# 1069066484/PanoSwinTransformerObjectDetection

Measured on AMD Instinct MI355X. Metric: panoramas/sec PanoSwin-T 512x1024 fwd+bwd, higher is better.
Workload: dtype bf16; 1 GPU; PanoSwin-T backbone (embed 96, depths 2-2-6-2, heads 3-6-12-24, ape, pano mode) fwd+bwd+AdamW on 3x512x1024 panoramas, BASELINE.json configs[1]; batch_per_gpu=8, global_batch=8, parallelism=dp1, hip_graph=True, overlap_allreduce=False, fused_window_attention=True, device=AMD Radeon Graphics

## Files before the change

### include/pswin.h

```cpp
#ifndef PSWIN_H_
#define PSWIN_H_

#include <stdint.h>

#ifdef __cplusplus
extern "C" {
#endif

#define PSWIN_ABI_VERSION 10

#define PSWIN_F32 0
#define PSWIN_BF16 1

#define PSWIN_MODE_PLANAR 0
#define PSWIN_MODE_PANO 1

#define PSWIN_OK 0
#define PSWIN_ERR_ARG (-1)
#define PSWIN_ERR_UNSUPPORTED (-2)

#define PSWIN_WS 7
#define PSWIN_WTOK 49
#define PSWIN_WPAD 64
#define PSWIN_HEAD_DIM 32
// ... 64 lines not shown
                         const float* ex_scale, int B, int S, int C, void* stream);

int pswin_ln_workspace(long long rows, int C);

int pswin_ln_partial_rows(long long rows, int C);
int pswin_ln_rows_tune(int mode);

int pswin_ln_patch_merge_fwd(const void* x, int x_dtype, const float* gamma, const float* beta, float eps, void* y,
                             int y_dtype, float* mean, float* rstd, int B, int H, int W, int C, void* stream);

int pswin_ln_patch_merge_bwd(const void* dy, int dy_dtype, const void* x, int x_dtype, const float* mean,
                             const float* rstd, const float* gamma, void* dx, float* dgamma, float* dbeta,
                             float* workspace, int B, int H, int W, int C, void* stream);

int pswin_patch_merge_gather(const void* x, int x_dtype, void* out, int out_dtype, int B, int H, int W, int C,
                             void* stream);

int pswin_patch_merge_scatter(const void* dout, int out_dtype, void* dx, int x_dtype, int B, int H, int W, int C,
                              void* stream);

int pswin_bn_workspace(int C);
int pswin_bn_relu_fwd(const void* y, int dtype, const float* gamma, const float* beta, const float* mean_offset,
                      float eps, float momentum, int train, float* running_mean, float* running_var, void* z, float* save_mean, float* save_rstd,
                      float* workspace, long long M, int C, void* stream);

int pswin_bn_relu_bwd(const void* dz, const void* y, int dtype, const float* gamma, const float* beta,
                      const float* save_mean, const float* save_rstd, int train, void* dy, float* dgamma, float* dbeta,
                      float* workspace, long long M, int C, void* stream);

int pswin_stem_workspace(int B, int H, int W);
int pswin_stem_pack_input(const float* x, int B, int H, int W, void* x4, void* stream);
int pswin_stem_conv1_stats(const void* x4, const void* w1p, int B, int H, int W, int want_xx, float* sums,
                           float* workspace, void* stream);
int pswin_stem_conv2_fwd(const void* x4, const void* w1p, const float* scale1, const float* shift1, const void* w2p, int B,
                         int H, int W, void* y2, float* sums2, float* workspace, void* stream);
int pswin_stem_conv3_fwd(const void* y2, const float* scale2, const float* shift2, const void* w3p, const float* bias3,
                         int B, int H, int W, void* tokens, void* stream);

int pswin_stem_conv3_bwd_stats(const void* dtok, const void* y2, const float* prm, const void* w3t, int B, int H, int W,
                               float* sums, float* workspace, void* stream);
int pswin_stem_conv3_bwd_data(const void* dtok, const void* y2, const float* prm, const void* w3t, int B, int H, int W,
                              void* dy2, void* stream);
int pswin_stem_conv3_wgrad(const void* dtok, const void* y2, const float* scale2, const float* shift2, int B, int H, int W,
                           const int32_t* perm, float* dw3, float* workspace, void* stream);
int pswin_stem_conv2_wgrad(const void* x4, const void* w1p, const float* scale1, const float* shift1, const void* dy2, int B,
                           int H, int W, const int32_t* perm, float* dw2, float* workspace, void* stream);
int pswin_stem_conv2_bwd(const void* x4, const void* w1p, const float* prm, const void* dy2, const void* w2t, int B, int H,
                         int W, float* out, float* workspace, void* stream);

int pswin_bias_gelu_fwd(const void* y, int dtype, const float* bias, void* h, long long M, int N, void* stream);
int pswin_bias_gelu_workspace(long long M, int N);
int pswin_bias_gelu_tune(int unr_fwd, int unr_bwd);
int pswin_bias_gelu_partial_rows(long long M, int N, int dtype);
int pswin_bias_gelu_bwd(const void* dh, const void* y, int dtype, const float* bias, void* dy, float* dbias,
                        float* workspace, long long M, int N, void* stream);

int pswin_stem_pack_weights(const float* w1, const float* w2, const float* w3, void* w1p, void* w2p, void* w2t, void* w3p,
                            void* w3t, void* stream);
int pswin_stem_bn_fold(const float* sum, const float* sumsq, double count, const float* gamma, const float* beta,
                       const float* conv_bias, float eps, float momentum, int training, float* running_mean,
                       float* running_var, int C, float* prm, long long* num_batches_tracked, void* stream);
int pswin_stem_bn2_coefs(const float* sums, const float* prm, double count, int training, float* prm5, void* stream);
int pswin_stem_conv1_wgrad(const float* out5, const float* xx, const void* w1p, const float* prm1, double count, int training,
                           float* dw1, float* db1, void* stream);

int pswin_gemm_tn_ring_supported(long long M, int N, int K);
int pswin_gemm_tn_ring_splits(long long M, int N, int K, int target_wgs);
int pswin_gemm_tn_ring(const void* dy, const void* x, void* partial, int partial_dtype, long long M, int N, int K, int splits, void* stream);
int pswin_gemm_tn_ring_bias(const void* dy, const void* x, void* partial, int partial_dtype, float* dbias_partial, int zero_lo, int zero_hi,
                            long long M, int N, int K, int splits, void* stream);

typedef struct pswin_tn_job {
    const void* dy;
    const void* x;
    void* partial;
    float* dbias_partial;
    long long M;
    int N, K, splits, partial_dtype, zero_lo, zero_hi;
    const float* sample_scale;
    int rows_per_sample;
} pswin_tn_job;
int pswin_gemm_tn_ring_jobs(const pswin_tn_job* jobs, int n_jobs, void* stream);
int pswin_gemm_tn_ring_table_bytes(void);

typedef struct pswin_transpose_job {
    const void* src;
    void* dst;
    int rows;
    int cols;
} pswin_transpose_job;
int pswin_transpose_jobs(const pswin_transpose_job* jobs, int n_jobs, void* stream);

int pswin_adamw_flat(float* p, const float* g, float* m, float* v, void* p_bf16, long long n, double lr, double beta1, double beta2, double eps,
                     double weight_decay, const float* step, void* stream);
#define PSWIN_ADAMW_MAX_GROUPS 8
int pswin_adamw_flat_groups(float* p, const float* g, float* m, float* v, void* p_bf16, long long n, const unsigned char* group_of,
                            int n_groups, const float* lr_mult, const float* decay_mult, double lr, double beta1, double beta2, double eps,
                            double weight_decay, const float* step, void* stream);

#define PSWIN_LR_FIXED 0
#define PSWIN_LR_STEP 1
#define PSWIN_WARMUP_NONE 0
#define PSWIN_WARMUP_CONSTANT 1
#define PSWIN_WARMUP_LINEAR 2
#define PSWIN_WARMUP_EXP 3
#define PSWIN_LR_MAX_MILESTONES 8
#define PSWIN_GRADSQ_PARTIALS 1024
typedef struct pswin_lr_schedule {
    int policy;
    int warmup;
    int warmup_iters;
    int by_epoch;
    int iters_per_epoch;
    int n_milestones;
    int step_every;
    int has_min_lr;
    int milestones[PSWIN_LR_MAX_MILESTONES];
    double warmup_ratio;
    double gamma;
    double min_lr;
} pswin_lr_schedule;
typedef struct pswin_step_record {
    double lr[PSWIN_ADAMW_MAX_GROUPS];
    double norm;
    float lr_base;
    float norm_f;
    float coef;
    float t;
    int applied;
    int iteration;
} pswin_step_record;
int pswin_grad_sumsq(const float* g, long long n, double* partials, void* stream);
int pswin_adamw_record(const double* partials, const pswin_lr_schedule* sched, double lr, int n_groups, const float* lr_mult,
                       double max_norm, int skip_nonfinite, float* step, float* iteration, float* skipped, pswin_step_record* record,
                       void* stream);
int pswin_adamw_flat_sched(float* p, const float* g, float* m, float* v, void* p_bf16, long long n, const unsigned char* group_of,
                           int n_groups, const float* decay_mult, double beta1, double beta2, double eps, double weight_decay,
                           const pswin_step_record* record, void* stream);
#define PSWIN_ROI_MAX_LEVELS 4
typedef struct pswin_roi_levels {
    const void* feat[PSWIN_ROI_MAX_LEVELS];
    float* dfeat[PSWIN_ROI_MAX_LEVELS];
    int H[PSWIN_ROI_MAX_LEVELS];
    int W[PSWIN_ROI_MAX_LEVELS];
    float spatial_scale[PSWIN_ROI_MAX_LEVELS];
    int n_levels;
} pswin_roi_levels;
int pswin_roi_align_supported(int C, int dtype);
int pswin_roi_align_fwd(const pswin_roi_levels* levels, const float* rois, const int32_t* roi_level, int R, int C, int P, int sampling_ratio,
                        int aligned, int dtype, void* out, void* stream);
int pswin_roi_align_bwd(const pswin_roi_levels* levels, const float* rois, const int32_t* roi_level, int R, int C, int P, int sampling_ratio,
                        int aligned, int dtype, const void* dout, void* stream);

int pswin_nms_workspace(int groups, int nmax);
int pswin_nms_groups(const float* boxes, const int32_t* counts, int groups, int nmax, float iou_threshold, unsigned char* keep, void* workspace,
                     void* stream);

int pswin_max_iou_assign_rows_per_workgroup(void);
int pswin_max_iou_assign_workspace(int B, int N, int Gmax);
int pswin_max_iou_assign(const float* cand, int cand_per_image, const float* gt, const int32_t* gt_count, int B, int N, int Gmax, int lead_gt,
                         float pos_iou_thr, float neg_iou_thr, float min_pos_iou, int match_low_quality, long long* gt_inds, float* max_iou,
                         void* workspace, void* stream);

int pswin_gemm_nt_supported(long long M, int K, int N);
int pswin_gemm_nt(const void* x, const void* w, const float* bias, void* y, long long M, int K, int N, int tile_m, void* stream);
int pswin_gemm_nt_f32(const void* x, const void* w, const float* bias, float* y, long long M, int K, int N, int tile_m, void* stream);
// ... 283 lines not shown
```

### panoswintransformerobjectdetection_amd/_lib.py

```python
import ctypes
import os

import torch

_PKG = os.path.dirname(os.path.abspath(__file__))
LIB_PATH = os.environ.get("PSWIN_LIB") or os.path.join(_PKG, "libpswin_hip.so")

F32, BF16 = 0, 1
MODE_PLANAR, MODE_PANO = 0, 1
WS, WTOK, WPAD, HEAD_DIM = 7, 49, 64, 32
ABI_VERSION = 10

_vp, _i, _f = ctypes.c_void_p, ctypes.c_int, ctypes.c_float
_ip = ctypes.POINTER(ctypes.c_int)

_PROTOTYPES = {
    "pswin_version": [],
    "pswin_window_grid": [_i, _i, _i, _ip, _ip, _ip],
    "pswin_window_map": [_i, _i, _i, _i, _vp, _vp, _vp],
    "pswin_planar_mask": [_i, _i, _i, _vp, _vp],
    "pswin_uv_grid": [_i, _i, _vp, _vp],
    "pswin_abs_pos_features": [_vp, _i, _vp, _vp],
    "pswin_gather_uv": [_vp, _vp, _i, _vp, _vp],
    "pswin_haversine_windows": [_vp, _vp, _i, _vp, _vp],
    "pswin_window_gather": [_vp, _i, _vp, _vp, _vp, _i, _i, _i, _i, _i, _vp],
    "pswin_window_scatter_add": [_vp, _i, _vp, _vp, _vp, _vp, _vp, _i, _i, _i, _i, _i, _vp],
    "pswin_ln_gather_fwd": [_vp, _i, _vp, _vp, _vp, _f, _vp, _i, _vp, _vp, _i, _i, _i, _i, _vp],
    "pswin_ln_gather_fwd_add": [_vp, _i, _vp, _vp, _vp, _f, _vp, _vp, _i, _vp, _vp, _i, _i, _i, _i, _vp],
    "pswin_ln_gather_bwd": [_vp, _i, _vp, _vp, _i, _vp, _vp, _vp, _vp, _vp, _vp, _vp, _vp, _vp, _vp, _i, _i, _i, _i, _vp],
    "pswin_ln_gather_bwd_ex": [_vp, _i, _vp, _vp, _i, _vp, _vp, _vp, _vp, _vp, _vp, _vp, _vp, _vp, _vp, _i, _i, _i, _i, _vp, _vp, _i, _vp, _vp, _i,
                               _vp],
    "pswin_scatter_add_ln_fwd": [_vp, _i, _vp, _vp, _vp, _vp, _vp, _vp, _vp, _f, _vp, _i, _vp, _vp, _i, _i, _i, _i, _vp],
    "pswin_scatter_add_ln_fwd_map": [_vp, _i, _vp, _vp, _vp, _vp, _vp, _vp, _vp, _f, _vp, _i, _vp, _vp, _i, _i, _i, _i, _vp, _i, _vp, _i, _vp],
    "pswin_ln_nchw_supported": [_i, _i],
    "pswin_ln_nchw_fwd": [_vp, _vp, _vp, _f, _vp, _vp, _vp, _i, _i, _i, _vp],
    "pswin_ln_nchw_bwd": [_vp, _vp, _vp, _vp, _vp, _vp, _vp, _vp, _vp, _vp, _i, _i, _i, _vp],
    "pswin_scatter_add_ln_nchw_fwd": [_vp, _vp, _vp, _vp, _vp, _vp, _vp, _f, _vp, _vp, _vp, _i, _i, _i, _vp],
    "pswin_ln_nchw_bwd_ex": [_vp, _vp, _vp, _vp, _vp, _vp, _vp, _vp, _vp, _vp, _vp, _vp, _i, _i, _i, _vp],
    "pswin_ln_workspace": [ctypes.c_longlong, _i],
    "pswin_ln_patch_merge_fwd": [_vp, _i, _vp, _vp, _f, _vp, _i, _vp, _vp, _i, _i, _i, _i, _vp],
    "pswin_ln_patch_merge_bwd": [_vp, _i, _vp, _i, _vp, _vp, _vp, _vp, _vp, _vp, _vp, _i, _i, _i, _i, _vp],
    "pswin_patch_merge_gather": [_vp, _i, _vp, _i, _i, _i, _i, _i, _vp],
    "pswin_patch_merge_scatter": [_vp, _i, _vp, _i, _i, _i, _i, _i, _vp],
    "pswin_bn_workspace": [_i],
    "pswin_bn_relu_fwd": [_vp, _i, _vp, _vp, _vp, _f, _f, _i, _vp, _vp, _vp, _vp, _vp, _vp, ctypes.c_longlong, _i, _vp],
    "pswin_bn_relu_bwd": [_vp, _vp, _i, _vp, _vp, _vp, _vp, _i, _vp, _vp, _vp, _vp, ctypes.c_longlong, _i, _vp],
    "pswin_stem_workspace": [_i, _i, _i],
    "pswin_stem_pack_input": [_vp, _i, _i, _i, _vp, _vp],
    "pswin_stem_conv1_stats": [_vp, _vp, _i, _i, _i, _i, _vp, _vp, _vp],
    "pswin_stem_conv2_fwd": [_vp, _vp, _vp, _vp, _vp, _i, _i, _i, _vp, _vp, _vp, _vp],
    "pswin_stem_conv3_fwd": [_vp, _vp, _vp, _vp, _vp, _i, _i, _i, _vp, _vp],
    "pswin_stem_conv3_bwd_stats": [_vp, _vp, _vp, _vp, _i, _i, _i, _vp, _vp, _vp],
    "pswin_stem_conv3_bwd_data": [_vp, _vp, _vp, _vp, _i, _i, _i, _vp, _vp],
    "pswin_stem_conv3_wgrad": [_vp, _vp, _vp, _vp, _i, _i, _i, _vp, _vp, _vp, _vp],
    "pswin_stem_conv2_wgrad": [_vp, _vp, _vp, _vp, _vp, _i, _i, _i, _vp, _vp, _vp, _vp],
    "pswin_stem_conv2_bwd": [_vp, _vp, _vp, _vp, _vp, _i, _i, _i, _vp, _vp, _vp],
    "pswin_stem_pack_weights": [_vp, _vp, _vp, _vp, _vp, _vp, _vp, _vp, _vp],
    "pswin_stem_bn_fold": [_vp, _vp, ctypes.c_double, _vp, _vp, _vp, _f, _f, _i, _vp, _vp, _i, _vp, _vp, _vp],
    "pswin_stem_bn2_coefs": [_vp, _vp, ctypes.c_double, _i, _vp, _vp],
    "pswin_stem_conv1_wgrad": [_vp, _vp, _vp, _vp, ctypes.c_double, _i, _vp, _vp, _vp],
    "pswin_gemm_tn_ring_supported": [ctypes.c_longlong, _i, _i],
    "pswin_gemm_tn_ring_splits": [ctypes.c_longlong, _i, _i, _i],
    "pswin_gemm_tn_ring": [_vp, _vp, _vp, _i, ctypes.c_longlong, _i, _i, _i, _vp],
    "pswin_gemm_tn_ring_bias": [_vp, _vp, _vp, _i, _vp, _i, _i, ctypes.c_longlong, _i, _i, _i, _vp],
    "pswin_gemm_tn_ring_jobs": [_vp, _i, _vp],
    "pswin_gemm_tn_ring_table_bytes": [],
    "pswin_transpose_jobs": [_vp, _i, _vp],
    "pswin_adamw_flat": [_vp, _vp, _vp, _vp, _vp, ctypes.c_longlong, ctypes.c_double, ctypes.c_double, ctypes.c_double, ctypes.c_double, ctypes.c_double, _vp, _vp],
    "pswin_adamw_flat_groups": [_vp, _vp, _vp, _vp, _vp, ctypes.c_longlong, _vp, _i, _vp, _vp, ctypes.c_double, ctypes.c_double,
                                ctypes.c_double, ctypes.c_double, ctypes.c_double, _vp, _vp],
    "pswin_grad_sumsq": [_vp, ctypes.c_longlong, _vp, _vp],
    "pswin_adamw_record": [_vp, _vp, ctypes.c_double, _i, _vp, ctypes.c_double, _i, _vp, _vp, _vp, _vp, _vp],
    "pswin_adamw_flat_sched": [_vp, _vp, _vp, _vp, _vp, ctypes.c_longlong, _vp, _i, _vp, ctypes.c_double, ctypes.c_double, ctypes.c_double,
                               ctypes.c_double, _vp, _vp],
    "pswin_roi_align_supported": [_i, _i],
    "pswin_roi_align_fwd": [_vp, _vp, _vp, _i, _i, _i, _i, _i, _i, _vp, _vp],
    "pswin_roi_align_bwd": [_vp, _vp, _vp, _i, _i, _i, _i, _i, _i, _vp, _vp],
    "pswin_nms_workspace": [_i, _i],
    "pswin_nms_groups": [_vp, _vp, _i, _i, ctypes.c_float, _vp, _vp, _vp],
    "pswin_max_iou_assign_rows_per_workgroup": [],
    "pswin_max_iou_assign_workspace": [_i, _i, _i],
    "pswin_max_iou_assign": [_vp, _i, _vp, _vp, _i, _i, _i, _i, _f, _f, _f, _i, _vp, _vp, _vp, _vp],
    "pswin_multiclass_nms_scores": [_vp, _i, _vp, _i, _i, _i, _f, _vp, _vp],
    "pswin_multiclass_nms_workspace": [_i, _i, _i],
    "pswin_multiclass_nms": [_vp, _vp, _vp, _vp, _i, _vp, _i, _i, _vp, _i, _i, _i, _f, _vp, _vp, _vp],
    "pswin_multiclass_nms_select": [_vp, _vp, ctypes.c_longlong, _i, _vp, _vp, _i, _vp, _i, _i, _vp, _i, _i, _i, _i, _vp, _vp, _vp, _vp, _vp, _vp],
    "pswin_paste_masks": [_vp, _i, ctypes.c_longlong, ctypes.c_longlong, ctypes.c_longlong, ctypes.c_longlong, _vp, _vp, _vp, _i, _i, _i, _i, _i,
                          _f, _vp, _vp],
    "pswin_aug_merge_proposals_launches": [_i, _i, _i],
    "pswin_aug_merge_proposals_workspace": [_i, _i, _i, _i],
    "pswin_aug_merge_proposals": [_vp, _vp, _vp, _vp, _i, _i, _i, _f, _i, _vp, _vp, _vp, _vp, _vp],
    "pswin_aug_map_rois": [_vp, _vp, _i, _i, _i, _vp, _vp],
    "pswin_aug_merge_bboxes": [_vp, _vp, _vp, _i, _i, _vp, _vp, _i, _i, _i, _i, _vp, _vp, _vp],
    "pswin_multiclass_nms_scores_boxes": [_vp, _vp, _i, _i, _i, _f, _vp, _vp],
    "pswin_multiclass_nms_boxes": [_vp, _vp, _vp, _i, _i, _i, _f, _vp, _vp, _vp],
    "pswin_multiclass_nms_select_boxes": [_vp, _vp, ctypes.c_longlong, _i, _vp, _i, _i, _i, _i, _vp, _vp, _vp, _vp, _vp, _vp],
    "pswin_paste_masks_aug": [_vp, _i, _vp, _vp, _vp, _i, _i, _i, _i, _i, _f, _vp, _vp],
    "pswin_rle_workspace": [ctypes.c_longlong, _i, _i, _vp],
    "pswin_rle_encode": [_vp, _vp, ctypes.c_longlong, _i, _i, _i, _vp, _vp, ctypes.c_longlong, _vp, _vp],
    "pswin_paste_masks_rle": [_vp, _i, ctypes.c_longlong, ctypes.c_longlong, ctypes.c_longlong, ctypes.c_longlong, _vp, _vp, _vp, _i, _i, _i, _i,
                              _i, _f, _vp, _vp, ctypes.c_longlong, _vp, _vp],
    "pswin_sample_rows_per_workgroup": [],
    "pswin_sample_workspace": [_i, _i, _i],
    "pswin_sample_ranks": [_vp, _vp, _i, _i, _i, _i, _vp, _vp, _vp, _vp],
    "pswin_rpn_targets": [_vp, _vp, _vp, _vp, _vp, _i, _i, _i, _i, _i, _vp, _vp, _vp, _vp, _vp],
    "pswin_roi_targets": [_vp, _vp, _vp, _vp, _vp, _vp, _i, _i, _i, _i, _i, _i, _vp, _vp, _vp, _vp, _vp, _vp, _vp],
    "pswin_mask_targets": [_vp, _vp, _vp, _vp, _i, _i, _i, _i, _i, _i, _vp, _vp],
    "pswin_rpn_proposals_rows_per_workgroup": [],
    "pswin_rpn_proposals_launches": [_vp, _i, _i, _i],
    "pswin_rpn_proposals_workspace": [_vp, _i, _i, _i, _i],
    "pswin_rpn_proposals": [_vp, _vp, _vp, _vp, _i, _i, _i, _f, _i, _i, _i, _vp, _vp, _vp, _vp, _vp],
    "pswin_cascade_rows_per_workgroup": [],
    "pswin_cascade_refine": [_vp, _vp, _i, _vp, _i, _vp, _i, _i, _i, _vp, _i, _i, _vp, _vp, _vp],
    "pswin_giou_rows_fwd": [_vp, _vp, _i, _vp, _vp, _vp, _i, _i, _vp, ctypes.c_double, _vp, _vp],
    "pswin_giou_rows_bwd": [_vp, _vp, _i, _vp, _vp, _vp, _vp, _i, _i, _vp, ctypes.c_double, _vp, _vp],
    "pswin_losses_rows_per_workgroup": [],
    "pswin_rpn_losses_chunk": [],
    "pswin_ce_rows_fwd": [_vp, _i, _vp, _i, _i, _vp, _vp],
    "pswin_ce_rows_bwd": [_vp, _i, _vp, _vp, _i, _i, _vp, _vp],
    "pswin_l1_rows_fwd": [_vp, _i, _vp, _vp, _vp, _i, _i, _vp, _vp],
    "pswin_l1_rows_bwd": [_vp, _i, _vp, _vp, _vp, _vp, _i, _i, _vp, _vp],
    "pswin_mask_bce_rows_fwd": [_vp, _i, ctypes.c_longlong, ctypes.c_longlong, ctypes.c_longlong, ctypes.c_longlong, _vp, _vp, _vp, _i, _i, _i,
                                _vp, _vp, _vp],
    "pswin_mask_bce_rows_bwd": [_vp, _i, ctypes.c_longlong, ctypes.c_longlong, ctypes.c_longlong, ctypes.c_longlong, _vp, _vp, _vp, _vp, _i, _i,
                                _i, _vp, _vp],
    "pswin_rpn_losses_fwd": [_vp, _vp, _vp, _vp, _vp, _vp, _i, _i, _i, _i, _vp, _vp],
    "pswin_rpn_losses_bwd": [_vp, _vp, _vp, _vp, _vp, _vp, _vp, _i, _i, _i, _i, _vp, _vp, _vp],
    "pswin_ap_segments_chunk": [],
    "pswin_box_iou_pairs": [_vp, _vp, _vp, _vp, _vp, _vp, _i, _i, _i, _vp, _vp, _vp, _vp],
    "pswin_mask_iou_workspace": [_i, _i, _i],
    "pswin_mask_iou_pairs": [_vp, _vp, _vp, _vp, _vp, _vp, _i, _i, _i, _i, _i, _vp, _vp, _vp, _vp, _vp],
    "pswin_eval_match": [_vp, _vp, _vp, _vp, _vp, _vp, _vp, _vp, _vp, _vp, _i, _vp, _i, _i, _i, _i, _i, _i, _vp, _vp, _vp, _vp, _vp, _vp, _vp,
                         _vp],
    "pswin_ap_segments": [_vp, _vp, _vp, _i, _i, _i, ctypes.c_longlong, _vp, _vp],
    "pswin_recall_match": [_vp, _vp, _vp, _vp, _vp, _vp, _i, _vp, _i, _i, _i, _i, _vp, _vp, _vp, _vp],
    "pswin_mask_inter_pairs": [_vp, _vp, _vp, _vp, _vp, _vp, _i, _i, _i, _i, _i, _vp, _vp, _vp],
    "pswin_coco_supported": [_i, _i, _i, _i, _i, _i],
    "pswin_coco_accumulate_chunk": [],
    "pswin_coco_match": [_vp, _vp, _vp, _vp, _vp, _vp, _vp, _vp, _vp, _vp, _vp, _vp, _i, _vp, _i, _i, _i, _i, _i, _i, _vp, _vp, _vp, _vp, _vp,
                         _vp, _vp, _vp, _vp],
    "pswin_coco_accumulate": [_vp, _vp, _vp, _vp, _vp, _i, _vp, _i, _i, _i, _i, ctypes.c_longlong, _vp, _vp, _vp],
    "pswin_gemm_nt_supported": [ctypes.c_longlong, _i, _i],
    "pswin_gemm_nt": [_vp, _vp, _vp, _vp, ctypes.c_longlong, _i, _i, _i, _vp],
    "pswin_gemm_nt_f32": [_vp, _vp, _vp, _vp, ctypes.c_longlong, _i, _i, _i, _vp],
    "pswin_gemm_nt_gelu_fwd": [_vp, _vp, _vp, _vp, _vp, ctypes.c_longlong, _i, _i, _i, _vp],
    "pswin_gemm_nt_partial_rows": [ctypes.c_longlong, _i],
    "pswin_gemm_nt_gelu_bwd": [_vp, _vp, _vp, _vp, _vp, _vp, ctypes.c_longlong, _i, _i, _i, _vp],
    "pswin_gemm_nt_live": [_vp, _vp, _vp, _vp, ctypes.c_longlong, _i, _i, _i, _vp, _i, _vp],
    "pswin_gemm_nt_gelu_fwd_live": [_vp, _vp, _vp, _vp, _vp, ctypes.c_longlong, _i, _i, _i, _vp, _i, _vp],
# ... 208 lines not shown
```

### panoswintransformerobjectdetection_amd/csrc/pswin_gemm_tn.hip

```cpp
#include <type_traits>

#include "pswin_common.hpp"

using namespace pswin;

namespace {

constexpr int MSTEP = 64, PANEL = 64 * 64 * 2;
using rsrc_t = __amdgpu_buffer_rsrc_t;
typedef __attribute__((address_space(3))) void lds_void;

constexpr int RING_THREADS = 512;
template <int WK, int WN, int STAGES>
struct RingGeom {
    static constexpr int PX = (96 * WK + 63) / 64, PD = (48 * WN + 63) / 64, PANELS = PX + PD, STAGE_BYTES = PANELS * PANEL;
    static constexpr int LOADS = PANELS;
    static constexpr int XWAVES = PX;
    static_assert(WK * WN == 8, "eight waves");
    static_assert((size_t)STAGES * STAGE_BYTES <= 160 * 1024, "LDS");
};

template <int OFF>
__device__ inline void ds_tr(u32x2& dst, unsigned addr) {
    asm volatile("ds_read_b64_tr_b16 %0, %1 offset:%2" : "=v"(dst) : "v"(addr), "i"(OFF) : "memory");
}
struct Frag {
    u32x2 lo, hi;
};
__device__ inline bf16x8 frag_bf16(const Frag& f) { return __builtin_bit_cast(bf16x8, u32x4{f.lo[0], f.lo[1], f.hi[0], f.hi[1]}); }
__device__ inline void wait_frags(Frag (&a)[6], Frag (&b)[3]) {
    asm volatile("s_waitcnt lgkmcnt(0)"
                 : "+v"(a[0].lo), "+v"(a[0].hi), "+v"(a[1].lo), "+v"(a[1].hi), "+v"(a[2].lo), "+v"(a[2].hi), "+v"(a[3].lo), "+v"(a[3].hi),
                   "+v"(a[4].lo), "+v"(a[4].hi), "+v"(a[5].lo), "+v"(a[5].hi), "+v"(b[0].lo), "+v"(b[0].hi), "+v"(b[1].lo), "+v"(b[1].hi),
                   "+v"(b[2].lo), "+v"(b[2].hi)
                 :
                 : "memory");
}

struct TnJob {
    const unsigned short* dy;
    const unsigned short* x;
    void* part;
    float* db;
    const float* sample_scale;
    int M, N, K, rows_per_split, zero_lo, zero_hi;
    int first_wg, flags, xmap, rows_per_sample;
};
constexpr int TN_JOBS_MAX = 48;
struct TnBatch {
    TnJob job[TN_JOBS_MAX];
    int n;
};
static_assert(sizeof(TnJob) == 80 && sizeof(TnBatch) <= 4000, "the job table travels in the 4 KB kernel-argument segment");

template <int WK, int WN, int STAGES>
__global__ __launch_bounds__(RING_THREADS, 2) void gemm_tn_ring_kernel(const TnBatch batch) {
    using G = RingGeom<WK, WN, STAGES>;
    int jlo = 0, jhi = batch.n - 1;
    while (jlo < jhi) {
        const int mid = (jlo + jhi + 1) >> 1;
        if (batch.job[mid].first_wg <= (int)blockIdx.x) jlo = mid;
        else jhi = mid - 1;
    }
    const TnJob& job = batch.job[jlo];
    const int jbid = (int)blockIdx.x - job.first_wg;
    const unsigned short* __restrict__ DY = job.dy;
    const unsigned short* __restrict__ X = job.x;
    void* __restrict__ P = job.part;
    float* __restrict__ DB = job.db;
    const int M = job.M, N = job.N, K = job.K, rows_per_split = job.rows_per_split;
    const int tiles_k = (K + 96 * WK - 1) / (96 * WK), tiles_n = (N + 48 * WN - 1) / (48 * WN);
    const int zero_lo = job.zero_lo, zero_hi = job.zero_hi;
    const bool out_bf16 = (job.flags & 1) != 0;
    constexpr int IA = 6, JB = 3;
    constexpr int RING_STAGE_BYTES = G::STAGE_BYTES, LOADS = G::LOADS;
    extern __shared__ __attribute__((aligned(1024))) char smem[];
    const int tid = threadIdx.x;
    const int wave = __builtin_amdgcn_readfirstlane(tid >> 6), lane = tid & 63;
    const int c = lane & 15, g = lane >> 4;
    const int wk = wave / WN, wn = wave - wk * WN;

    int split, tk, tn;
    {
        const int xm = job.xmap, g = xm & 255, gn = (xm >> 8) & 255, bk = (xm >> 16) & 255, bn = (xm >> 24) & 255;
        const int xcd = jbid & 7, loc = jbid >> 3, lane = xcd / g, blk = xcd - lane * g, ik = blk / gn, in = blk - ik * gn;
        const int per = bk * bn, round = loc / per, within = loc - round * per, wk_ = within / bn;
        split = round * (8 / g) + lane;
        tk = ik * bk + wk_;
        tn = in * bn + (within - wk_ * bn);
        if (split >= (job.flags >> 1) || tk >= tiles_k || tn >= tiles_n) return;
    }
    const int k0 = tk * (96 * WK), n0 = tn * (48 * WN);
    const int m_begin = split * rows_per_split;
    int steps = rows_per_split / MSTEP;
    {
        const int left = (M - m_begin + MSTEP - 1) / MSTEP;
        steps = left < steps ? (left > 0 ? left : 0) : steps;
    }
    const float* __restrict__ SS = job.sample_scale;
    unsigned long long live_slabs = 0ull;
    if (SS != nullptr) {
        const int rows_per_sample = job.rows_per_sample;
        const unsigned long long live_samples = live_sample_mask(SS, M / rows_per_sample);
        bool live = false;
        if (lane < steps) {
            const int r0 = m_begin + lane * MSTEP, r1 = (r0 + MSTEP < M ? r0 + MSTEP : M) - 1;
            const int s0 = r0 / rows_per_sample, s1 = r1 / rows_per_sample;
            const unsigned long long span = s1 - s0 >= 63 ? ~0ull : (2ull << (s1 - s0)) - 1ull;
            live = ((live_samples >> s0) & span) != 0ull;
        }
        const unsigned long long b = __ballot(live);
        live_slabs = (unsigned long long)(unsigned)__builtin_amdgcn_readfirstlane((int)(unsigned)b) |
                     (unsigned long long)(unsigned)__builtin_amdgcn_readfirstlane((int)(unsigned)(b >> 32)) << 32;
        steps = __builtin_popcountll(live_slabs);
    }

    static_assert((G::PX * 8) % LOADS == 0, "a wave's blocks must not straddle the two operands");
    const bool mine_x = wave * LOADS < G::PX * 8;
    const rsrc_t src = mine_x ? __builtin_amdgcn_make_buffer_rsrc(const_cast<unsigned short*>(X), 0, (int)((size_t)M * K * 2), 0x00020000)
                              : __builtin_amdgcn_make_buffer_rsrc(const_cast<unsigned short*>(DY), 0, (int)((size_t)M * N * 2), 0x00020000);
    const unsigned ld2 = (unsigned)((mine_x ? K : N) * 2);
    const int c0 = mine_x ? k0 : n0;
    const int lr = lane >> 3, pch = lane & 7;
    unsigned goff[8];
    const int last_panel = ((mine_x ? K : N) - c0 + 63) / 64 - 1;
#pragma unroll
    for (int j = 0; j < LOADS; ++j) {
        const int blk_all = wave * LOADS + j - (mine_x ? 0 : G::PX * 8), blk = blk_all & 7;
        int panel = blk_all >> 3;
        panel = panel > last_panel ? (last_panel > 0 ? last_panel : 0) : panel;
        const int row = 8 * blk + lr;
        const int f = ((row >> 1) & 1) | (((row >> 3) & 1) << 1);
        const int col = (((pch >> 1) ^ f) << 4) + ((pch & 1) << 3);
        goff[j] = (unsigned)row * ld2 + (unsigned)((c0 + 64 * panel + col) * 2);
    }
    auto issue = [&](int step, int stage) {
        char* base = smem + stage * RING_STAGE_BYTES + wave * LOADS * 1024;
        int slab = step;
        if (SS != nullptr) {
            slab = __builtin_ctzll(live_slabs);
            live_slabs &= live_slabs - 1ull;
        }
        const unsigned m = (unsigned)(m_begin + slab * MSTEP) * ld2;
#pragma unroll
        for (int j = 0; j < LOADS; ++j) __builtin_amdgcn_raw_ptr_buffer_load_lds(src, (lds_void*)(base + j * 1024), 16, goff[j] + m, 0, 0, 0);
    };

    f32x4 acc[IA][JB];
#pragma unroll
    for (int i = 0; i < IA; ++i)
#pragma unroll
        for (int j = 0; j < JB; ++j) acc[i][j] = f32x4{0.f, 0.f, 0.f, 0.f};
    const bool sum_db = DB != nullptr && tk == 0 && wk == 0;
    f32x4 accs[JB];
#pragma unroll
    for (int j = 0; j < JB; ++j) accs[j] = f32x4{0.f, 0.f, 0.f, 0.f};
    const bf16x8 ones = __builtin_bit_cast(bf16x8, u32x4{0x3F803F80u, 0x3F803F80u, 0x3F803F80u, 0x3F803F80u});

    const int q = c >> 2, p8 = c & 3;
    const int fl = ((q >> 1) & 1) | ((g & 1) << 1);
    const unsigned lds0 = (unsigned)(size_t)(lds_void*)smem;
    const unsigned lane_row = lds0 + (unsigned)((8 * g + q) * 128 + p8 * 8);
    unsigned xoff[4];
#pragma unroll
    for (int cb = 0; cb < 4; ++cb) xoff[cb] = ((unsigned)(cb ^ fl) << 5) + lane_row;
    unsigned abase[IA], bbase[JB];
#pragma unroll
    for (int i = 0; i < IA; ++i) {
        const int col0 = wk * 96 + 16 * i;
        abase[i] = xoff[(col0 >> 4) & 3] + (unsigned)((col0 >> 6) * PANEL);
    }
#pragma unroll
    for (int j = 0; j < JB; ++j) {
        const int col0 = wn * 48 + 16 * j;
        bbase[j] = xoff[(col0 >> 4) & 3] + (unsigned)((col0 >> 6) * PANEL + G::PX * PANEL);
    }
    auto read_n = [&](auto ks_tag, auto n_tag, unsigned stage_off, Frag (&a)[6], Frag (&b)[3]) {
        constexpr int KS = decltype(ks_tag)::value, NN = decltype(n_tag)::value, F = NN >> 1, OFF = KS * 4096 + (NN & 1) * 512;
        if constexpr (F < 6) {
            if constexpr (NN & 1) ds_tr<OFF>(a[F].hi, abase[F] + stage_off);
            else ds_tr<OFF>(a[F].lo, abase[F] + stage_off);
        } else {
            if constexpr (NN & 1) ds_tr<OFF>(b[F - 6].hi, bbase[F - 6] + stage_off);
            else ds_tr<OFF>(b[F - 6].lo, bbase[F - 6] + stage_off);
        }
    };
    auto mma_n = [&](auto n_tag, const bf16x8 (&af)[6], const bf16x8 (&bfr)[3]) {
        constexpr int NN = decltype(n_tag)::value, I = NN % 6, J = NN / 6;
        acc[I][J] = mfma32(af[I], bfr[J], acc[I][J]);
    };
    auto phase = [&](auto ks_tag, auto read_tag, unsigned stage_off, Frag (&cur_a)[6], Frag (&cur_b)[3], Frag (&nxt_a)[6], Frag (&nxt_b)[3]) {
        constexpr bool READ = decltype(read_tag)::value;
        bf16x8 af[IA], bfr[JB];
#pragma unroll
        for (int i = 0; i < IA; ++i) af[i] = frag_bf16(cur_a[i]);
#pragma unroll
        for (int j = 0; j < JB; ++j) bfr[j] = frag_bf16(cur_b[j]);
        auto slot = [&](auto n_tag) {
            if constexpr (READ) read_n(ks_tag, n_tag, stage_off, nxt_a, nxt_b);
            mma_n(n_tag, af, bfr);
            __builtin_amdgcn_sched_barrier(0);
        };
        [&]<int... Ns>(std::integer_sequence<int, Ns...>) { (slot(std::integral_constant<int, Ns>{}), ...); }(std::make_integer_sequence<int, 18>{});
        if (sum_db) {
#pragma unroll
            for (int j = 0; j < JB; ++j) accs[j] = mfma32(ones, bfr[j], accs[j]);
        }
    };
    auto read_all = [&](auto ks_tag, unsigned stage_off, Frag (&a)[6], Frag (&b)[3]) {
        [&]<int... Ns>(std::integer_sequence<int, Ns...>) { (read_n(ks_tag, std::integral_constant<int, Ns>{}, stage_off, a, b), ...); }(std::make_integer_sequence<int, 18>{});
    };
    using KS0 = std::integral_constant<int, 0>;
    using KS1 = std::integral_constant<int, 1>;

    static_assert(STAGES == 2 || STAGES == 3, "");
    static_assert(STAGES == 2 || LOADS == 6, "the counted wait below is written out for 6 loads per slab");
    if (steps > 0) issue(0, 0);
    if (STAGES == 3 && steps > 1) issue(1, 1);
    Frag a0[6], b0[3], a1[6], b1[3];
    int stage = 0;
    for (int st = 0; st < steps; ++st) {
        if (STAGES == 3 && st + 1 < steps) asm volatile("s_waitcnt vmcnt(6)" ::: "memory");
        else asm volatile("s_waitcnt vmcnt(0)" ::: "memory");
        if (st > 0) wait_frags(a1, b1);
        __builtin_amdgcn_s_barrier();
        const unsigned stage_off = (unsigned)(stage * RING_STAGE_BYTES);
        if (st + STAGES - 1 < steps) issue(st + STAGES - 1, stage == 0 ? STAGES - 1 : stage - 1);
        if (st == 0) {
            read_all(KS0{}, stage_off, a0, b0);
        } else {
            phase(KS0{}, std::true_type{}, stage_off, a1, b1, a0, b0);
        }
        wait_frags(a0, b0);
        __builtin_amdgcn_sched_barrier(0);
        phase(KS1{}, std::true_type{}, stage_off, a0, b0, a1, b1);
        stage = stage == STAGES - 1 ? 0 : stage + 1;
    }
    if (steps > 0) {
        wait_frags(a1, b1);
        __builtin_amdgcn_sched_barrier(0);
        phase(KS0{}, std::false_type{}, 0u, a1, b1, a0, b0);
    }

    if (sum_db && g == 0) {
#pragma unroll
        for (int j = 0; j < JB; ++j) {
            const int n = n0 + wn * 48 + 16 * j + c;
            if (n < N) DB[(size_t)split * N + n] = (n >= zero_lo && n < zero_hi) ? 0.f : accs[j][0];
        }
    }
#pragma unroll
    for (int j = 0; j < JB; ++j) {
        const int n = n0 + wn * 48 + 16 * j + c;
        if (n >= N) continue;
#pragma unroll
        for (int i = 0; i < IA; ++i) {
            const int k = k0 + wk * 96 + 16 * i + 4 * g;
            if (k >= K) continue;
            const size_t o = (size_t)split * N * K + (size_t)n * K + k;
            if (out_bf16) {
                *reinterpret_cast<u32x2*>(reinterpret_cast<unsigned short*>(P) + o) = u32x2{pack2_bf16(acc[i][j][0], acc[i][j][1]), pack2_bf16(acc[i][j][2], acc[i][j][3])};
            } else {
                *reinterpret_cast<f32x4*>(reinterpret_cast<float*>(P) + o) = acc[i][j];
            }
        }
    }
}

inline int ring_geom(int N, int K) {
    if (N >= 192 && K >= 192 && N % 192 == 0 && K % 192 == 0) return 0;
    if (K == 96 && N >= 48 && N <= 384 && N % 16 == 0) return 1;
    if (K == 384 && N == 96) return 2;
    return -1;
}

template <int WK, int WN, int STAGES>
int launch_tn_batch(const TnBatch& b, int wgs, hipStream_t st) {
    using G = RingGeom<WK, WN, STAGES>;
    constexpr size_t lds = (size_t)STAGES * G::STAGE_BYTES;
    static std::atomic<unsigned long long> configured{0};
    if (const int rc = ensure_dynamic_lds(reinterpret_cast<const void*>(&gemm_tn_ring_kernel<WK, WN, STAGES>), lds, configured)) return rc;
    hipLaunchKernelGGL((gemm_tn_ring_kernel<WK, WN, STAGES>), dim3(wgs), dim3(RING_THREADS), lds, st, b);
    PSWIN_LAUNCH_RET();
}

inline bool tn_job_ok(const pswin_tn_job& q) {
    return q.dy && q.x && q.partial && q.M >= 64 && (q.M + 64) * (long long)(q.K > q.N ? q.K : q.N) * 2 < 0xFFFFFF00ll && ring_geom(q.N, q.K) >= 0 &&
           q.splits >= 1 && q.splits <= q.M / 64 && valid_dtype(q.partial_dtype) && aligned16(q.dy) && aligned16(q.x) && aligned16(q.partial) &&
           q.zero_lo >= 0 && q.zero_hi >= q.zero_lo && q.zero_hi <= q.N &&
           (!q.sample_scale || (q.rows_per_sample > 0 && q.M % q.rows_per_sample == 0 && q.M / q.rows_per_sample <= LIVE_SAMPLES_MAX &&
                                (q.M + q.splits - 1) / q.splits <= 64 * MSTEP));
}

int launch_tn_jobs(const pswin_tn_job* jobs, int n_jobs, int geom, hipStream_t st) {
    TnBatch b;
    b.n = 0;
    long long wgs = 0;
    auto flush = [&]() -> int {
        if (b.n == 0) return PSWIN_OK;
        int rc;
        if (geom == 0) rc = launch_tn_batch<2, 4, 3>(b, (int)wgs, st);
        else if (geom == 1) rc = launch_tn_batch<1, 8, 2>(b, (int)wgs, st);
        else rc = launch_tn_batch<4, 2, 2>(b, (int)wgs, st);
        b.n = 0;
        wgs = 0;
        return rc;
    };
    for (int i = 0; i < n_jobs; ++i) {
        const pswin_tn_job& q = jobs[i];
        if (ring_geom(q.N, q.K) != geom) continue;
        const int tk = geom == 0 ? 192 : (geom == 1 ? 96 : 384), tn = geom == 0 ? 192 : (geom == 1 ? 384 : 96);
        TnJob& j = b.job[b.n];
        j.dy = reinterpret_cast<const unsigned short*>(q.dy);
        j.x = reinterpret_cast<const unsigned short*>(q.x);
        j.part = q.partial;
        j.db = q.dbias_partial;
        j.M = (int)q.M;
        j.N = q.N;
        j.K = q.K;
        const int tiles_k = (q.K + tk - 1) / tk, tiles_n = (q.N + tn - 1) / tn;
        j.sample_scale = q.sample_scale;
        j.rows_per_sample = q.sample_scale ? q.rows_per_sample : 0;
        j.rows_per_split = (int)(((q.M + q.splits - 1) / q.splits + MSTEP - 1) / MSTEP * MSTEP);
        j.zero_lo = q.zero_lo;
        j.zero_hi = q.zero_hi;
        j.first_wg = (int)wgs;
        int n_wg;
        {
            const int S = q.splits;
            int g = 1;
            if (S < 8) {
                int p2 = 1;
                while (p2 < S) p2 *= 2;
                g = 8 / p2;
            }
            int best_gn = 1;
            long long best = -1;
            for (int gn = 1; gn <= g; gn *= 2) {
                const int gk = g / gn;
                const long long cost = (long long)((tiles_k + gk - 1) / gk) * tk + (long long)((tiles_n + gn - 1) / gn) * tn;
                if (best < 0 || cost < best) best = cost, best_gn = gn;
            }
            const int gn = best_gn, gk = g / gn, bk = (tiles_k + gk - 1) / gk, bn = (tiles_n + gn - 1) / gn;
            const int lanes = 8 / g, rounds = (S + lanes - 1) / lanes;
            j.xmap = g | gn << 8 | bk << 16 | bn << 24;
            n_wg = 8 * rounds * bk * bn;
        }
        j.flags = (q.partial_dtype == PSWIN_BF16 ? 1 : 0) | q.splits << 1;
        wgs += n_wg;
        if (++b.n == TN_JOBS_MAX || wgs > (1ll << 24)) {
            if (const int rc = flush()) return rc;
        }
    }
    return flush();
}

}

extern "C" {

int pswin_gemm_tn_ring_supported(long long M, int N, int K) {
    return M >= 64 && (M + 64) * (long long)(K > N ? K : N) * 2 < 0xFFFFFF00ll && ring_geom(N, K) >= 0;
}

int pswin_gemm_tn_ring_splits(long long M, int N, int K, int target_wgs) {
    if (!pswin_gemm_tn_ring_supported(M, N, K)) return PSWIN_ERR_ARG;
    const int geom = ring_geom(N, K);
    const int tiles = geom == 0 ? (N / 192) * (K / 192) : 1;
    if (target_wgs <= 0) target_wgs = 256;
    int s = target_wgs / tiles;
    const int smax = (int)(M / 256) > 0 ? (int)(M / 256) : 1;
    if (s > smax) s = smax;
    return s < 1 ? 1 : s;
}

int pswin_gemm_tn_ring_table_bytes(void) { return (int)sizeof(TnBatch); }

int pswin_gemm_tn_ring_jobs(const pswin_tn_job* jobs, int n_jobs, void* stream) {
    PSWIN_CHECK_ARG(jobs && n_jobs > 0);
    for (int i = 0; i < n_jobs; ++i) PSWIN_CHECK_ARG(tn_job_ok(jobs[i]));
    for (int geom = 0; geom < 3; ++geom)
        if (const int rc = launch_tn_jobs(jobs, n_jobs, geom, (hipStream_t)stream)) return rc;
    return PSWIN_OK;
}

int pswin_gemm_tn_ring_bias(const void* dy, const void* x, void* partial, int partial_dtype, float* dbias_partial, int zero_lo, int zero_hi, long long M,
                            int N, int K, int splits, void* stream) {
    pswin_tn_job q;
    q.dy = dy;
    q.x = x;
    q.partial = partial;
    q.dbias_partial = dbias_partial;
    q.M = M;
    q.N = N;
    q.K = K;
    q.splits = splits;
    q.partial_dtype = partial_dtype;
    q.zero_lo = zero_lo;
    q.zero_hi = zero_hi;
    q.sample_scale = nullptr;
    q.rows_per_sample = 0;
    return pswin_gemm_tn_ring_jobs(&q, 1, stream);
}

int pswin_gemm_tn_ring(const void* dy, const void* x, void* partial, int partial_dtype, long long M, int N, int K, int splits, void* stream) {
    return pswin_gemm_tn_ring_bias(dy, x, partial, partial_dtype, nullptr, 0, 0, M, N, K, splits, stream);
}

}
```

Measured before the change: 885.7 panoramas/s.

## Merge all wgrad ring geometries into one launch with job reordering

Replaces the per-geometry template kernels with a single kernel that dispatches on geometry packed into each job's xmap, so all TN wgrad jobs go out in one launch instead of up to three. Jobs are sorted by rows per split, longest first. An optional env-gated mode splits the work into two queues and interleaves them by proportional block share. A host-side plan API is added for inspection. In exchange, every geometry now reserves the largest LDS ring and the fused kernel may hold more registers, which can lower occupancy for the smaller geometries.

```diff
diff --git a/include/pswin.h b/include/pswin.h
--- a/include/pswin.h
+++ b/include/pswin.h
@@ -170,6 +170,7 @@
 } pswin_tn_job;
 int pswin_gemm_tn_ring_jobs(const pswin_tn_job* jobs, int n_jobs, void* stream);
 int pswin_gemm_tn_ring_table_bytes(void);
+int pswin_gemm_tn_ring_plan(const pswin_tn_job* jobs, int n_jobs, int interleave, int* plan, int cap, int* n_launches);
 
 typedef struct pswin_transpose_job {
     const void* src;
diff --git a/panoswintransformerobjectdetection_amd/_lib.py b/panoswintransformerobjectdetection_amd/_lib.py
--- a/panoswintransformerobjectdetection_amd/_lib.py
+++ b/panoswintransformerobjectdetection_amd/_lib.py
@@ -65,6 +65,7 @@
     "pswin_gemm_tn_ring_bias": [_vp, _vp, _vp, _i, _vp, _i, _i, ctypes.c_longlong, _i, _i, _i, _vp],
     "pswin_gemm_tn_ring_jobs": [_vp, _i, _vp],
     "pswin_gemm_tn_ring_table_bytes": [],
+    "pswin_gemm_tn_ring_plan": [_vp, _i, _i, _vp, _i, _vp],
     "pswin_transpose_jobs": [_vp, _i, _vp],
     "pswin_adamw_flat": [_vp, _vp, _vp, _vp, _vp, ctypes.c_longlong, ctypes.c_double, ctypes.c_double, ctypes.c_double, ctypes.c_double, ctypes.c_double, _vp, _vp],
     "pswin_adamw_flat_groups": [_vp, _vp, _vp, _vp, _vp, ctypes.c_longlong, _vp, _i, _vp, _vp, ctypes.c_double, ctypes.c_double,
diff --git a/panoswintransformerobjectdetection_amd/csrc/pswin_gemm_tn.hip b/panoswintransformerobjectdetection_amd/csrc/pswin_gemm_tn.hip
--- a/panoswintransformerobjectdetection_amd/csrc/pswin_gemm_tn.hip
+++ b/panoswintransformerobjectdetection_amd/csrc/pswin_gemm_tn.hip
@@ -1,4 +1,8 @@
+#include <algorithm>
+#include <cstdlib>
+#include <cstring>
 #include <type_traits>
+#include <vector>
 
 #include "pswin_common.hpp"
 
@@ -43,35 +47,64 @@
     void* part;
     float* db;
     const float* sample_scale;
-    int M, N, K, rows_per_split, zero_lo, zero_hi;
-    int first_wg, flags, xmap, rows_per_sample;
+    int M, N, K, splits, zero_lo, zero_hi;
+    int first_wg, xmap;
 };
-constexpr int TN_JOBS_MAX = 48;
+__host__ __device__ inline int tn_xmap(int lg, int lgn, int geom, int out_bf16, int samples, int bk, int bn) {
+    return lg | lgn << 2 | geom << 4 | out_bf16 << 6 | samples << 7 | bk << 16 | bn << 24;
+}
+__host__ __device__ inline int tn_rows_per_split(int M, int splits) { return ((M + splits - 1) / splits + MSTEP - 1) / MSTEP * MSTEP; }
+__host__ __device__ inline int tn_tile_k(int geom) { return geom == 0 ? 192 : (geom == 1 ? 96 : 384); }
+__host__ __device__ inline int tn_tile_n(int geom) { return geom == 0 ? 192 : (geom == 1 ? 384 : 96); }
+
+constexpr int TN_JOBS_MAX = 54;
 struct TnBatch {
     TnJob job[TN_JOBS_MAX];
-    int n;
+    int n, n0, blocks0, blocks1;
+    unsigned share;
 };
-static_assert(sizeof(TnJob) == 80 && sizeof(TnBatch) <= 4000, "the job table travels in the 4 KB kernel-argument segment");
-
-template <int WK, int WN, int STAGES>
-__global__ __launch_bounds__(RING_THREADS, 2) void gemm_tn_ring_kernel(const TnBatch batch) {
-    using G = RingGeom<WK, WN, STAGES>;
-    int jlo = 0, jhi = batch.n - 1;
+static_assert(sizeof(TnJob) == 72 && sizeof(TnBatch) <= 4000, "the job table travels in the 4 KB kernel-argument segment");
+
+__host__ __device__ inline int tn_queue1_before(int b, int blocks0, int blocks1, unsigned share) {
+    const long long h = (long long)(((unsigned long long)(unsigned)b * share + 32768ull) >> 16), lo = b - blocks0;
+    const long long c = h < lo ? lo : h;
+    return (int)(c > blocks1 ? blocks1 : c);
+}
+__host__ __device__ inline int tn_find_job(const TnBatch& batch, int wg, int& jbid) {
+    const int b = wg >> 3;
+    const int h0 = tn_queue1_before(b, batch.blocks0, batch.blocks1, batch.share), h1 = tn_queue1_before(b + 1, batch.blocks0, batch.blocks1, batch.share);
+    const bool q1 = h1 != h0;
+    const int qwg = (q1 ? h0 : b - h0) << 3 | (wg & 7);
+    int jlo = q1 ? batch.n0 : 0, jhi = (q1 ? batch.n : batch.n0) - 1;
     while (jlo < jhi) {
         const int mid = (jlo + jhi + 1) >> 1;
-        if (batch.job[mid].first_wg <= (int)blockIdx.x) jlo = mid;
+        if (batch.job[mid].first_wg <= qwg) jlo = mid;
         else jhi = mid - 1;
     }
-    const TnJob& job = batch.job[jlo];
-    const int jbid = (int)blockIdx.x - job.first_wg;
+    jbid = qwg - batch.job[jlo].first_wg;
+    return jlo;
+}
+__host__ __device__ inline bool tn_slot(int xm, int splits, int tiles_k, int tiles_n, int jbid, int& split, int& tk, int& tn) {
+    const int g = 1 << (xm & 3), gn = 1 << ((xm >> 2) & 3), bk = (xm >> 16) & 255, bn = (xm >> 24) & 255;
+    const int xcd = jbid & 7, loc = jbid >> 3, lane = xcd / g, blk = xcd - lane * g, ik = blk / gn, in = blk - ik * gn;
+    const int per = bk * bn, round = loc / per, within = loc - round * per, wk_ = within / bn;
+    split = round * (8 / g) + lane;
+    tk = ik * bk + wk_;
+    tn = in * bn + (within - wk_ * bn);
+    return split < splits && tk < tiles_k && tn < tiles_n;
+}
+
+template <int WK, int WN, int STAGES>
+__device__ __forceinline__ void gemm_tn_ring_body(const TnJob& job, const int jbid) {
+    using G = RingGeom<WK, WN, STAGES>;
     const unsigned short* __restrict__ DY = job.dy;
     const unsigned short* __restrict__ X = job.x;
     void* __restrict__ P = job.part;
     float* __restrict__ DB = job.db;
-    const int M = job.M, N = job.N, K = job.K, rows_per_split = job.rows_per_split;
+    const int M = job.M, N = job.N, K = job.K, rows_per_split = tn_rows_per_split(M, job.splits);
     const int tiles_k = (K + 96 * WK - 1) / (96 * WK), tiles_n = (N + 48 * WN - 1) / (48 * WN);
     const int zero_lo = job.zero_lo, zero_hi = job.zero_hi;
-    const bool out_bf16 = (job.flags & 1) != 0;
+    const bool out_bf16 = (job.xmap >> 6 & 1) != 0;
     constexpr int IA = 6, JB = 3;
     constexpr int RING_STAGE_BYTES = G::STAGE_BYTES, LOADS = G::LOADS;
     extern __shared__ __attribute__((aligned(1024))) char smem[];
@@ -81,15 +114,7 @@
     const int wk = wave / WN, wn = wave - wk * WN;
 
     int split, tk, tn;
-    {
-        const int xm = job.xmap, g = xm & 255, gn = (xm >> 8) & 255, bk = (xm >> 16) & 255, bn = (xm >> 24) & 255;
-        const int xcd = jbid & 7, loc = jbid >> 3, lane = xcd / g, blk = xcd - lane * g, ik = blk / gn, in = blk - ik * gn;
-        const int per = bk * bn, round = loc / per, within = loc - round * per, wk_ = within / bn;
-        split = round * (8 / g) + lane;
-        tk = ik * bk + wk_;
-        tn = in * bn + (within - wk_ * bn);
-        if (split >= (job.flags >> 1) || tk >= tiles_k || tn >= tiles_n) return;
-    }
+    if (!tn_slot(job.xmap, job.splits, tiles_k, tiles_n, jbid, split, tk, tn)) return;
     const int k0 = tk * (96 * WK), n0 = tn * (48 * WN);
     const int m_begin = split * rows_per_split;
     int steps = rows_per_split / MSTEP;
@@ -100,8 +125,8 @@
     const float* __restrict__ SS = job.sample_scale;
     unsigned long long live_slabs = 0ull;
     if (SS != nullptr) {
-        const int rows_per_sample = job.rows_per_sample;
-        const unsigned long long live_samples = live_sample_mask(SS, M / rows_per_sample);
+        const int samples = job.xmap >> 7 & 127, rows_per_sample = M / samples;
+        const unsigned long long live_samples = live_sample_mask(SS, samples);
         bool live = false;
         if (lane < steps) {
             const int r0 = m_begin + lane * MSTEP, r1 = (r0 + MSTEP < M ? r0 + MSTEP : M) - 1;
@@ -267,92 +292,114 @@
     }
 }
 
+__global__ __launch_bounds__(RING_THREADS, 2) void gemm_tn_ring_kernel(const TnBatch batch) {
+    int jbid;
+    const TnJob& job = batch.job[tn_find_job(batch, (int)blockIdx.x, jbid)];
+    const int geom = job.xmap >> 4 & 3;
+    if (geom == 0) gemm_tn_ring_body<2, 4, 3>(job, jbid);
+    else if (geom == 1) gemm_tn_ring_body<1, 8, 2>(job, jbid);
+    else gemm_tn_ring_body<4, 2, 2>(job, jbid);
+}
+constexpr size_t RING_LDS = 3 * RingGeom<2, 4, 3>::STAGE_BYTES;
+static_assert(RING_LDS >= 2 * RingGeom<1, 8, 2>::STAGE_BYTES && RING_LDS >= 2 * RingGeom<4, 2, 2>::STAGE_BYTES, "the largest ring");
+
 inline int ring_geom(int N, int K) {
-    if (N >= 192 && K >= 192 && N % 192 == 0 && K % 192 == 0) return 0;
+    if (N >= 192 && K >= 192 && N % 192 == 0 && K % 192 == 0 && N <= 255 * 192 && K <= 255 * 192) return 0;
     if (K == 96 && N >= 48 && N <= 384 && N % 16 == 0) return 1;
     if (K == 384 && N == 96) return 2;
     return -1;
 }
 
-template <int WK, int WN, int STAGES>
 int launch_tn_batch(const TnBatch& b, int wgs, hipStream_t st) {
-    using G = RingGeom<WK, WN, STAGES>;
-    constexpr size_t lds = (size_t)STAGES * G::STAGE_BYTES;
     static std::atomic<unsigned long long> configured{0};
-    if (const int rc = ensure_dynamic_lds(reinterpret_cast<const void*>(&gemm_tn_ring_kernel<WK, WN, STAGES>), lds, configured)) return rc;
-    hipLaunchKernelGGL((gemm_tn_ring_kernel<WK, WN, STAGES>), dim3(wgs), dim3(RING_THREADS), lds, st, b);
+    if (const int rc = ensure_dynamic_lds(reinterpret_cast<const void*>(&gemm_tn_ring_kernel), RING_LDS, configured)) return rc;
+    hipLaunchKernelGGL(gemm_tn_ring_kernel, dim3(wgs), dim3(RING_THREADS), RING_LDS, st, b);
     PSWIN_LAUNCH_RET();
 }
 
-inline bool tn_job_ok(const pswin_tn_job& q) {
-    return q.dy && q.x && q.partial && q.M >= 64 && (q.M + 64) * (long long)(q.K > q.N ? q.K : q.N) * 2 < 0xFFFFFF00ll && ring_geom(q.N, q.K) >= 0 &&
-           q.splits >= 1 && q.splits <= q.M / 64 && valid_dtype(q.partial_dtype) && aligned16(q.dy) && aligned16(q.x) && aligned16(q.partial) &&
-           q.zero_lo >= 0 && q.zero_hi >= q.zero_lo && q.zero_hi <= q.N &&
+inline bool tn_shape_ok(const pswin_tn_job& q) {
+    return q.M >= 64 && (q.M + 64) * (long long)(q.K > q.N ? q.K : q.N) * 2 < 0xFFFFFF00ll && ring_geom(q.N, q.K) >= 0 && q.splits >= 1 &&
+           q.splits <= q.M / 64 && q.zero_lo >= 0 && q.zero_hi >= q.zero_lo && q.zero_hi <= q.N &&
            (!q.sample_scale || (q.rows_per_sample > 0 && q.M % q.rows_per_sample == 0 && q.M / q.rows_per_sample <= LIVE_SAMPLES_MAX &&
                                 (q.M + q.splits - 1) / q.splits <= 64 * MSTEP));
 }
-
-int launch_tn_jobs(const pswin_tn_job* jobs, int n_jobs, int geom, hipStream_t st) {
+inline bool tn_job_ok(const pswin_tn_job& q) {
+    return q.dy && q.x && q.partial && valid_dtype(q.partial_dtype) && aligned16(q.dy) && aligned16(q.x) && aligned16(q.partial) && tn_shape_ok(q);
+}
+
+int tn_fill_job(const pswin_tn_job& q, int first_wg, TnJob& j) {
+    const int geom = ring_geom(q.N, q.K), tk = tn_tile_k(geom), tn = tn_tile_n(geom);
+    j.dy = reinterpret_cast<const unsigned short*>(q.dy);
+    j.x = reinterpret_cast<const unsigned short*>(q.x);
+    j.part = q.partial;
+    j.db = q.dbias_partial;
+    j.sample_scale = q.sample_scale;
+    j.M = (int)q.M;
+    j.N = q.N;
+    j.K = q.K;
+    j.splits = q.splits;
+    j.zero_lo = q.zero_lo;
+    j.zero_hi = q.zero_hi;
+    j.first_wg = first_wg;
+    const int tiles_k = (q.K + tk - 1) / tk, tiles_n = (q.N + tn - 1) / tn;
+    const int S = q.splits;
+    int g = 1, lg = 0;
+    if (S < 8) {
+        int p2 = 1;
+        while (p2 < S) p2 *= 2;
+        g = 8 / p2;
+        while ((1 << lg) < g) ++lg;
+    }
+    int best_lgn = 0;
+    long long best = -1;
+    for (int lgn = 0; lgn <= lg; ++lgn) {
+        const int gn = 1 << lgn, gk = g / gn;
+        const long long cost = (long long)((tiles_k + gk - 1) / gk) * tk + (long long)((tiles_n + gn - 1) / gn) * tn;
+        if (best < 0 || cost < best) best = cost, best_lgn = lgn;
+    }
+    const int gn = 1 << best_lgn, gk = g / gn, bk = (tiles_k + gk - 1) / gk, bn = (tiles_n + gn - 1) / gn;
+    const int lanes = 8 / g, rounds = (S + lanes - 1) / lanes;
+    j.xmap = tn_xmap(lg, best_lgn, geom, q.partial_dtype == PSWIN_BF16 ? 1 : 0, q.sample_scale ? (int)(q.M / q.rows_per_sample) : 0, bk, bn);
+    return 8 * rounds * bk * bn;
+}
+
+bool tn_interleave_enabled() {
+    const char* e = std::getenv("PSWIN_WGRAD_INTERLEAVE");
+    return e && e[0] == '1' && e[1] == 0;
+}
+
+template <typename F>
+int tn_for_each_launch(const pswin_tn_job* jobs, int n_jobs, bool interleave, F&& launch) {
+    std::vector<int> order(n_jobs);
+    for (int i = 0; i < n_jobs; ++i) order[i] = i;
+    std::stable_sort(order.begin(), order.end(), [&](int a, int b) { return jobs[a].M / jobs[a].splits > jobs[b].M / jobs[b].splits; });
     TnBatch b;
-    b.n = 0;
-    long long wgs = 0;
-    auto flush = [&]() -> int {
-        if (b.n == 0) return PSWIN_OK;
-        int rc;
-        if (geom == 0) rc = launch_tn_batch<2, 4, 3>(b, (int)wgs, st);
-        else if (geom == 1) rc = launch_tn_batch<1, 8, 2>(b, (int)wgs, st);
-        else rc = launch_tn_batch<4, 2, 2>(b, (int)wgs, st);
+    std::memset(&b, 0, sizeof(b));
+    int src[TN_JOBS_MAX];
+    for (int i0 = 0; i0 < n_jobs;) {
+        int i1 = i0;
+        TnJob scratch;
+        for (long long wgs = 0; i1 < n_jobs && i1 - i0 < TN_JOBS_MAX && wgs <= (1ll << 24); ++i1) wgs += tn_fill_job(jobs[order[i1]], 0, scratch);
+        int q_wgs[2] = {0, 0};
         b.n = 0;
-        wgs = 0;
-        return rc;
-    };
-    for (int i = 0; i < n_jobs; ++i) {
-        const pswin_tn_job& q = jobs[i];
-        if (ring_geom(q.N, q.K) != geom) continue;
-        const int tk = geom == 0 ? 192 : (geom == 1 ? 96 : 384), tn = geom == 0 ? 192 : (geom == 1 ? 384 : 96);
-        TnJob& j = b.job[b.n];
-        j.dy = reinterpret_cast<const unsigned short*>(q.dy);
-        j.x = reinterpret_cast<const unsigned short*>(q.x);
-        j.part = q.partial;
-        j.db = q.dbias_partial;
-        j.M = (int)q.M;
-        j.N = q.N;
-        j.K = q.K;
-        const int tiles_k = (q.K + tk - 1) / tk, tiles_n = (q.N + tn - 1) / tn;
-        j.sample_scale = q.sample_scale;
-        j.rows_per_sample = q.sample_scale ? q.rows_per_sample : 0;
-        j.rows_per_split = (int)(((q.M + q.splits - 1) / q.splits + MSTEP - 1) / MSTEP * MSTEP);
-        j.zero_lo = q.zero_lo;
-        j.zero_hi = q.zero_hi;
-        j.first_wg = (int)wgs;
-        int n_wg;
-        {
-            const int S = q.splits;
-            int g = 1;
-            if (S < 8) {
-                int p2 = 1;
-                while (p2 < S) p2 *= 2;
-                g = 8 / p2;
+        for (int q = 0; q < 2; ++q) {
+            if (q == 1) b.n0 = b.n;
+            for (int t = i0; t < i1; ++t) {
+                const pswin_tn_job& job = jobs[order[t]];
+                if ((interleave && ring_geom(job.N, job.K) != 0) != (q == 1)) continue;
+                src[b.n] = order[t];
+                q_wgs[q] += tn_fill_job(job, q_wgs[q], b.job[b.n]);
+                ++b.n;
             }
-            int best_gn = 1;
-            long long best = -1;
-            for (int gn = 1; gn <= g; gn *= 2) {
-                const int gk = g / gn;
-                const long long cost = (long long)((tiles_k + gk - 1) / gk) * tk + (long long)((tiles_n + gn - 1) / gn) * tn;
-                if (best < 0 || cost < best) best = cost, best_gn = gn;
-            }
-            const int gn = best_gn, gk = g / gn, bk = (tiles_k + gk - 1) / gk, bn = (tiles_n + gn - 1) / gn;
-            const int lanes = 8 / g, rounds = (S + lanes - 1) / lanes;
-            j.xmap = g | gn << 8 | bk << 16 | bn << 24;
-            n_wg = 8 * rounds * bk * bn;
-        }
-        j.flags = (q.partial_dtype == PSWIN_BF16 ? 1 : 0) | q.splits << 1;
-        wgs += n_wg;
-        if (++b.n == TN_JOBS_MAX || wgs > (1ll << 24)) {
-            if (const int rc = flush()) return rc;
-        }
-    }
-    return flush();
+        }
+        b.blocks0 = q_wgs[0] >> 3;
+        b.blocks1 = q_wgs[1] >> 3;
+        const long long blocks = (long long)b.blocks0 + b.blocks1;
+        b.share = (unsigned)((((long long)b.blocks1 << 16) + blocks / 2) / blocks);
+        if (const int rc = launch(b, src, q_wgs[0] + q_wgs[1])) return rc;
+        i0 = i1;
+    }
+    return PSWIN_OK;
 }
 
 }
@@ -379,9 +426,32 @@
 int pswin_gemm_tn_ring_jobs(const pswin_tn_job* jobs, int n_jobs, void* stream) {
     PSWIN_CHECK_ARG(jobs && n_jobs > 0);
     for (int i = 0; i < n_jobs; ++i) PSWIN_CHECK_ARG(tn_job_ok(jobs[i]));
-    for (int geom = 0; geom < 3; ++geom)
-        if (const int rc = launch_tn_jobs(jobs, n_jobs, geom, (hipStream_t)stream)) return rc;
-    return PSWIN_OK;
+    return tn_for_each_launch(jobs, n_jobs, tn_interleave_enabled(),
+                              [&](const TnBatch& b, const int*, int wgs) { return launch_tn_batch(b, wgs, (hipStream_t)stream); });
+}
+
+int pswin_gemm_tn_ring_plan(const pswin_tn_job* jobs, int n_jobs, int interleave, int* plan, int cap, int* n_launches) {
+    PSWIN_CHECK_ARG(jobs && n_jobs > 0 && cap >= 0 && (plan || cap == 0));
+    for (int i = 0; i < n_jobs; ++i) PSWIN_CHECK_ARG(tn_shape_ok(jobs[i]));
+    long long total = 0;
+    int launches = 0;
+    const int rc = tn_for_each_launch(jobs, n_jobs, interleave < 0 ? tn_interleave_enabled() : interleave != 0, [&](const TnBatch& b, const int* src, int wgs) {
+        for (int w = 0; w < wgs; ++w, ++total) {
+            if (total >= cap) continue;
+            int jbid, split, tk, tn;
+            const int t = tn_find_job(b, w, jbid);
+            const TnJob& j = b.job[t];
+            const int geom = j.xmap >> 4 & 3, tiles_k = (j.K + tn_tile_k(geom) - 1) / tn_tile_k(geom), tiles_n = (j.N + tn_tile_n(geom) - 1) / tn_tile_n(geom);
+            const bool works = tn_slot(j.xmap, j.splits, tiles_k, tiles_n, jbid, split, tk, tn);
+            int* o = plan + 4 * total;
+            o[0] = works ? src[t] : -1, o[1] = split, o[2] = tk, o[3] = tn;
+        }
+        ++launches;
+        return (int)PSWIN_OK;
+    });
+    if (rc) return rc;
+    if (n_launches) *n_launches = launches;
+    return total > 0x7FFFFFFFll ? PSWIN_ERR_ARG : (int)total;
 }
 
 int pswin_gemm_tn_ring_bias(const void* dy, const void* x, void* partial, int partial_dtype, float* dbias_partial, int zero_lo, int zero_hi, long long M,
```

Measured after the change: 886.3 panoramas/s (median of 2 runs). About the same (+0.1%).
